# alazarteka/Self-Forcing

Measured on AMD Instinct MI355X. Metric: decoded frames/sec/node, Wan-1.3B 832x480 4-step AR rollout, higher is better.
Workload: dtype bf16

## Files before the change

self-forcing_amd/csrc/dit_forward.hip:

```cpp
#include <algorithm>
#include "sf_host.h"

int sf_internal_write_kv_indices(void* buf, int layers, int64_t global_end, int64_t local_end, void* stream);

namespace {

struct Work {
  void *x, *xn, *qkv, *q, *att, *hbuf, *cols, *headout, *sin, *etmp, *e, *e0, *ctx1, *ctx;
  void* xq;
  float* xs;
  size_t total;
};

constexpr int FP8_MAX_SEGMENTS = 8;

Work carve(const sf_model* m, void* ws, int B, int F, int lat_h, int lat_w, int groups) {
  const size_t M = (size_t)B * F * (lat_h / 2) * (lat_w / 2);
  const size_t C = m->dim, BG = (size_t)B * groups, T = (size_t)B * m->text_len;
  Carve c(ws);
  Work w;
  w.x = c.take(M * C * 2);
  w.xn = c.take(M * C * 2);
  w.qkv = c.take(M * 3 * C * 2);
  w.q = c.take(M * C * 2);
// ... 34 lines not shown
  w.t1 = c.take(R * im->clip_dim * 2);
  w.ctx = c.take(2 * R * (size_t)m->dim * 2);
  w.total = c.off;
  return w;
}

}

extern "C" size_t sf_dit_workspace_bytes(const sf_model* model, const sf_i2v_model* i2v_model, int batch, int frames, int lat_h, int lat_w,
                                         int groups) {
  if (!model || batch <= 0 || frames <= 0 || lat_h <= 0 || lat_w <= 0 || groups <= 0) return 0;
  const size_t base = carve(model, nullptr, batch, frames, lat_h, lat_w, groups).total;
  if (!i2v_model) return base;
  if (!base || i2v_model->clip_len <= 0 || i2v_model->clip_dim <= 0) return 0;
  return carve_img(model, i2v_model, nullptr, base, batch).total;
}

extern "C" int sf_dit_forward(const sf_model* m, const sf_forward_call* call, void* stream) {
  SF_CHECK(m && call, "sf_dit_forward: null argument");
  const sf_forward_args* const* ps = call->passes;
  const int np = call->n_passes;
  SF_CHECK(np == 1 || np == 2, "sf_dit_forward: one or two passes per call (n_passes=%d)", np);
  const sf_forward_args* a = ps[0];
  SF_CHECK(a && ps[np - 1], "sf_dit_forward: null argument");
  SF_CHECK(ps[np - 1]->workspace == a->workspace && ps[np - 1]->workspace_bytes == a->workspace_bytes,
           "sf_dit_forward: both passes name the same workspace (sized for 2 x batch)");
  int32_t* const cross_keys = call->cross_keys;
  float* const cross_log2w = call->cross_log2w;
  SF_CHECK((cross_keys == nullptr) == (cross_log2w == nullptr), "sf_dit_forward: cross_keys and cross_log2w come together");
  const sf_i2v_model* const im = call->i2v_model;
// ... 120 lines not shown
      void* ctx_img = (void*)bptr(iw.ctx, (size_t)R * C);
      SF_TRY(sf_layernorm_rows(ia->clip_feature, im->img_ln0_w, im->img_ln0_b, iw.t0, R, D, im->img_eps, stream));
      SF_TRY(Gemm(iw.t0, D, im->img_fc1_w, D, iw.t1, D, R, D, D).bias(im->img_fc1_b).bf16(stream));
      SF_TRY(sf_clip_gelu(iw.t1, iw.t1, (int64_t)R * D, stream));
      SF_TRY(Gemm(iw.t1, D, im->img_fc2_w, D, ctx_raw, C, R, C, D).bias(im->img_fc2_b).bf16(stream));
      SF_TRY(sf_layernorm_affine(ctx_raw, im->img_ln1_w, im->img_ln1_b, ctx_img, R, C, im->img_eps, stream));
      for (int l = 0; l < m->num_layers; ++l) {
        const sf_i2v_layer& il = im->layers_host[l];
        SF_TRY(Gemm(ctx_img, C, il.kvimg_w, C, ia->kimg_cache_host[l], C, R, C, C).bias(il.kvimg_b).bf16(stream));
        SF_TRY(sf_rmsnorm(ia->kimg_cache_host[l], C, il.norm_k_img_w, ia->kimg_cache_host[l], C, R, C, m->eps, stream));
        SF_TRY(Gemm(ctx_img, C, bptr(il.kvimg_w, (size_t)C * C), C, ia->vimg_cache_host[l], C, R, C, C).bias(bptr(il.kvimg_b, C)).bf16(stream));
      }
    }
  }

  for (int l = 0; l < m->num_layers; ++l) {
    const sf_layer_weights& lw = m->layers_host[l];
    const sf_layer_fp8& lq = f8 ? m->layers_fp8_host[l] : no_fp8;
    const void* mod = lw.modulation;
    const bool last_layer = l == m->num_layers - 1;
    SF_TRY(sf_layernorm_modulate(ws.x, ws.xn, Mt, C, m->eps, bptr(mod, 0), bptr(mod, C), bptr(ws.e0, 0), bptr(ws.e0, C), 6L * C, rpg, stream));
    SF_TRY(lin(Gemm(ws.xn, C, lw.qkv_w, C, ws.qkv, 3 * C, Mt, 3 * C, C).bias(lw.qkv_b).fp8w(lq.qkv_q, lq.qkv_s, M)));
    for (int p = 0; p < np; ++p) {
      const sf_forward_args* q = ps[p];
      const size_t roff = (size_t)p * M;
      if (q->evict > 0) {
        SF_TRY(sf_kv_evict(q->k_cache_host[l], B, q->cache_tokens, C, q->sink_tokens, q->evict, q->keep, q->evict_scratch, q->evict_scratch_bytes, stream));
        SF_TRY(sf_kv_evict(q->v_cache_host[l], B, q->cache_tokens, C, q->sink_tokens, q->evict, q->keep, q->evict_scratch, q->evict_scratch_bytes, stream));
      }
      SF_TRY(sf_qkv_norm_rope_cache(bptr(ws.qkv, roff * 3 * C), lw.norm_q_w, lw.norm_k_w, (void*)bptr(ws.q, roff * C), q->k_cache_host[l], q->v_cache_host[l],
                                    m->rope_cos, m->rope_sin, B, F, h, w, C, m->num_heads, q->cache_tokens, q->write_start, q->start_frame, m->eps, stream));
      if (q->cache_only && last_layer) continue;
      SF_TRY(Attention(bptr(ws.q, roff * C), C, (long)L * C, bptr(q->k_cache_host[l], (size_t)q->attn_start * C), bptr(q->v_cache_host[l], (size_t)q->attn_start * C),
                       C, cache_b, (void*)bptr(ws.att, roff * C), C, (long)L * C, B, m->num_heads, L, q->attn_end - q->attn_start).run(stream));
    }
    const int p0 = last_layer ? first_full : 0;
    if (p0 == np) return finish_indices();
    const size_t r0 = (size_t)p0 * M;
    const int Mr = (np - p0) * M;
    void* x = (void*)bptr(ws.x, r0 * C);
    void* xn = (void*)bptr(ws.xn, r0 * C);
    void* qb = (void*)bptr(ws.q, r0 * C);
    void* att = (void*)bptr(ws.att, r0 * C);
    void* hb = (void*)bptr(ws.hbuf, r0 * m->ffn_dim);
    const void* e0r = bptr(ws.e0, (size_t)p0 * BG * 6 * C);
    SF_TRY(lin(Gemm(att, C, lw.o_w, C, x, C, Mr, C, C).bias(lw.o_b).epi(SF_EPI_BIAS_GATE_RESID).resid(x, C)
// ... 33 lines not shown
```

self-forcing_amd/csrc/elementwise.hip:

```cpp
#include "sf_common.h"
#include "../../include/sf_hip.h"

namespace {

constexpr int ROWS_PER_BLOCK = 4;

template <int NCH>
__device__ __forceinline__ void load_row(const bf16_t* row, int lane, float (&v)[NCH][8]) {
#pragma unroll
  for (int i = 0; i < NCH; ++i) {
    const bf16x8 t = *reinterpret_cast<const bf16x8*>(row + (i * 64 + lane) * 8);
#pragma unroll
    for (int j = 0; j < 8; ++j) v[i][j] = (float)t[j];
  }
}

template <int NCH>
__device__ __forceinline__ void ln_stats(const float (&v)[NCH][8], int C, float eps, float& mean, float& rstd) {
  float s = 0.f;
#pragma unroll
  for (int i = 0; i < NCH; ++i)
#pragma unroll
    for (int j = 0; j < 8; ++j) s += v[i][j];
  mean = wave_sum(s) / (float)C;
// ... 88 lines not shown
  for (int i = 0; i < NCH; ++i)
#pragma unroll
    for (int j = 0; j < 8; ++j) q += v[i][j] * v[i][j];
  const float r = rsqrtf(wave_sum(q) / (float)C + eps);
#pragma unroll
  for (int i = 0; i < NCH; ++i) {
    const int e = (i * 64 + lane) * 8;
    const bf16x8 wt = *reinterpret_cast<const bf16x8*>(w + e);
    bf16x8 o;
#pragma unroll
    for (int j = 0; j < 8; ++j) o[j] = (bf16_t)((float)(bf16_t)(v[i][j] * r) * (float)wt[j]);
    *reinterpret_cast<bf16x8*>(out + (long)row * ldo + e) = o;
  }
}

template <int NCH>
__global__ __launch_bounds__(256) void qkv_norm_rope_cache_kernel(
    const bf16_t* __restrict__ qkv, const bf16_t* __restrict__ wq, const bf16_t* __restrict__ wk,
    bf16_t* __restrict__ q_out, bf16_t* __restrict__ k_cache, bf16_t* __restrict__ v_cache,
    const float* __restrict__ rope_cos, const float* __restrict__ rope_sin, int rows, int L, int hgt, int wid, int C,
    long cache_tokens, int write_start, int start_frame, float eps, int c0, int c1) {
  const int lane = threadIdx.x & 63;
  const int row = blockIdx.x * ROWS_PER_BLOCK + (threadIdx.x >> 6);
  if (row >= rows) return;
  const int b = row / L, t = row - b * L;
  const int fi = t / (hgt * wid), rem = t - fi * (hgt * wid);
  const int hi = rem / wid, wi = rem - hi * wid;
  const int pos_t = start_frame + fi;
  const bf16_t* src = qkv + (long)row * 3 * C;
  const long crow = ((long)b * cache_tokens + write_start + t) * C;

#pragma unroll
  for (int i = 0; i < NCH; ++i) {
    const int e = (i * 64 + lane) * 8;
    *reinterpret_cast<u32x4*>(v_cache + crow + e) = *reinterpret_cast<const u32x4*>(src + 2 * C + e);
  }

#pragma unroll
  for (int which = 0; which < 2; ++which) {
    float v[NCH][8];
    load_row<NCH>(src + which * C, lane, v);
    float q = 0.f;
#pragma unroll
    for (int i = 0; i < NCH; ++i)
#pragma unroll
      for (int j = 0; j < 8; ++j) q += v[i][j] * v[i][j];
    const float r = rsqrtf(wave_sum(q) / (float)C + eps);
    const bf16_t* wn = which ? wk : wq;
    bf16_t* dst = which ? (k_cache + crow) : (q_out + (long)row * C);
#pragma unroll
    for (int i = 0; i < NCH; ++i) {
      const int e = (i * 64 + lane) * 8;
      const bf16x8 wt = *reinterpret_cast<const bf16x8*>(wn + e);
      const int pair0 = (e & 127) >> 1;
// ... 206 lines not shown
extern "C" int sf_rmsnorm(const void* x, int ldx, const void* weight, void* out, int ldo, int M, int C, float eps,
                          void* stream) {
  SF_CHECK(x && out && weight, "sf_rmsnorm: null tensor");
  SF_CHECK(M > 0 && channels_ok(C) && ldx >= C && ldo >= C && ldx % 8 == 0 && ldo % 8 == 0, "sf_rmsnorm: unsupported shape M=%d C=%d", M, C);
  const dim3 grid((M + ROWS_PER_BLOCK - 1) / ROWS_PER_BLOCK), block(256);
  hipStream_t s = (hipStream_t)stream;
  switch (C / 512) {
#define SF_RMS_CASE(N) \
  case N: return sf_launch<&rmsnorm_kernel<N>>("sf_rmsnorm", grid, block, 0, s, (const bf16_t*)x, ldx, (const bf16_t*)weight, (bf16_t*)out, ldo, M, C, eps);
    SF_RMS_CASE(1) SF_RMS_CASE(2) SF_RMS_CASE(3) SF_RMS_CASE(4) SF_RMS_CASE(5) SF_RMS_CASE(6) SF_RMS_CASE(8) SF_RMS_CASE(10)
#undef SF_RMS_CASE
    default: SF_CHECK(false, "sf_rmsnorm: unsupported channel count %d", C);
  }
}

extern "C" int sf_qkv_norm_rope_cache(const void* qkv, const void* norm_q_w, const void* norm_k_w, void* q_out,
                                      void* k_cache, void* v_cache, const float* rope_cos, const float* rope_sin,
                                      int B, int f, int h, int w, int C, int num_heads, int64_t cache_tokens,
                                      int write_start, int start_frame, float eps, void* stream) {
  SF_CHECK(qkv && norm_q_w && norm_k_w && q_out && k_cache && v_cache && rope_cos && rope_sin, "sf_qkv_norm_rope_cache: null tensor");
  SF_CHECK(B > 0 && f > 0 && h > 0 && w > 0 && channels_ok(C), "sf_qkv_norm_rope_cache: unsupported shape");
  SF_CHECK(num_heads > 0 && C == num_heads * 128, "sf_qkv_norm_rope_cache: head_dim must be 128 (C=%d heads=%d)", C, num_heads);
  const int L = f * h * w;
  SF_CHECK(write_start >= 0 && (int64_t)write_start + L <= cache_tokens, "sf_qkv_norm_rope_cache: cache overflow: write_start=%d + L=%d > capacity=%lld",
           write_start, L, (long long)cache_tokens);
  SF_CHECK(start_frame >= 0 && start_frame + f <= 1024 && h <= 1024 && w <= 1024, "sf_qkv_norm_rope_cache: RoPE position out of the 1024-entry table");
  const int rows = B * L;
  const dim3 grid((rows + ROWS_PER_BLOCK - 1) / ROWS_PER_BLOCK), block(256);
  hipStream_t s = (hipStream_t)stream;
  const int c = 64, c1 = c / 3, c0 = c - 2 * c1;
  switch (C / 512) {
#define SF_QKV_CASE(N)                                                                                                                         \
  case N: return sf_launch<&qkv_norm_rope_cache_kernel<N>>("sf_qkv_norm_rope_cache", grid, block, 0, s, (const bf16_t*)qkv, (const bf16_t*)norm_q_w, \
                             (const bf16_t*)norm_k_w, (bf16_t*)q_out, (bf16_t*)k_cache, (bf16_t*)v_cache, rope_cos, rope_sin,                    \
                             rows, L, h, w, C, (long)cache_tokens, write_start, start_frame, eps, c0, c1);
    SF_QKV_CASE(1) SF_QKV_CASE(2) SF_QKV_CASE(3) SF_QKV_CASE(4) SF_QKV_CASE(5) SF_QKV_CASE(6) SF_QKV_CASE(8) SF_QKV_CASE(10)
#undef SF_QKV_CASE
    default: SF_CHECK(false, "sf_qkv_norm_rope_cache: unsupported channel count %d", C);
  }
}

extern "C" int sf_kv_evict(void* cache, int B, int64_t cache_tokens, int row_elems, int sink, int evict, int keep,
                           void* scratch, size_t scratch_bytes, void* stream) {
  SF_CHECK(cache && B > 0 && row_elems > 0 && (row_elems % 8) == 0, "sf_kv_evict: bad arguments");
  SF_CHECK(sink >= 0 && evict >= 0 && keep >= 0 && (int64_t)sink + evict + keep <= cache_tokens, "sf_kv_evict: window out of range");
  if (evict == 0 || keep == 0) return 0;
  const long row_b = (long)row_elems * 2;
  const long bytes = (long)keep * row_b;
  SF_CHECK(scratch && scratch_bytes >= (size_t)(bytes * B), "sf_kv_evict: scratch too small (%zu < %ld)", scratch_bytes, bytes * B);
  char* base = (char*)cache;
  const long bstride = (long)cache_tokens * row_b;
  const int gx = (int)min((long)2048, (bytes / 16 + 255) / 256);
  const dim3 grid(gx, B), block(256);
  hipStream_t s = (hipStream_t)stream;
// ... 122 lines not shown
```

self-forcing_amd/csrc/gemm_bf16.hip:

```cpp
#include <type_traits>
#include "sf_common.h"
#include "lds_dma.h"
#include "../../include/sf_hip.h"

namespace {

constexpr int BM = 128, BN = 128, BK = 64;
constexpr int GEMM_THREADS = 256;
constexpr int TILE_BYTES = BM * BK * 2;
constexpr int STAGE_BYTES = 2 * TILE_BYTES;
constexpr int GEMM_LDS = 2 * STAGE_BYTES;

struct GemmP {
  const bf16_t* a;
  const bf16_t* w;
  const bf16_t* bias;
  bf16_t* out;
  const bf16_t* resid;
  const bf16_t* gate_mod;
  const bf16_t* gate_e0;
  long gate_group_stride;
  int rows_per_group;
  int M, N, K, lda, ldw, ldo, ldr;
  int tiles_m, tiles_n;
  long a_bs, w_bs, o_bs, r_bs;
  const float* a_scale;
  const float* w_scale;
  int rows_per_seg;
};

typedef int i32x4 __attribute__((ext_vector_type(4)));
typedef int i32x8 __attribute__((ext_vector_type(8)));

__device__ __forceinline__ f32x4 mfma_f8(const bf16x8& w0, const bf16x8& w1, const bf16x8& x0, const bf16x8& x1, const f32x4& acc) {
  const i32x8 wv = __builtin_shufflevector(__builtin_bit_cast(i32x4, w0), __builtin_bit_cast(i32x4, w1), 0, 1, 2, 3, 4, 5, 6, 7);
  const i32x8 xv = __builtin_shufflevector(__builtin_bit_cast(i32x4, x0), __builtin_bit_cast(i32x4, x1), 0, 1, 2, 3, 4, 5, 6, 7);
  return __builtin_amdgcn_mfma_scale_f32_16x16x128_f8f6f4(wv, xv, acc, 0, 0, 0, 127, 0, 127);
}

template <int MT>
__device__ __forceinline__ void fp8_scale_acc(const GemmP& p, f32x4 (&acc)[MT][4], int m_base, int n_base, int lane) {
  f32x4 ws[4];
#pragma unroll
  for (int nt = 0; nt < 4; ++nt) ws[nt] = *reinterpret_cast<const f32x4*>(p.w_scale + min(n_base + nt * 16 + (lane >> 4) * 4, p.N - 4));
// ... 58 lines not shown
  __device__ __forceinline__ bf16x4 bias() const { return *reinterpret_cast<const bf16x4*>(p.bias + n); }
  __device__ __forceinline__ bf16x4 gate_mod() const { return *reinterpret_cast<const bf16x4*>(p.gate_mod + n); }
  __device__ __forceinline__ bf16x4 gate_e0() const { return *reinterpret_cast<const bf16x4*>(e0row + n); }
  __device__ __forceinline__ bf16x4 resid() const { return *reinterpret_cast<const bf16x4*>(p.resid + (long)m * p.ldr + n); }
};

struct EpiRegs {
  bf16x4 b, gm, ge, rv;
  __device__ __forceinline__ bool has_bias() const { return true; }
  __device__ __forceinline__ bf16x4 bias() const { return b; }
  __device__ __forceinline__ bf16x4 gate_mod() const { return gm; }
  __device__ __forceinline__ bf16x4 gate_e0() const { return ge; }
  __device__ __forceinline__ bf16x4 resid() const { return rv; }
};

template <int EPI, int MT>
__device__ __forceinline__ void gemm_epilogue(const GemmP& p, f32x4 (&acc)[MT][4], int mrow, int ncol) {
#pragma unroll
  for (int mt = 0; mt < MT; ++mt) {
    const int m = mrow + mt * 16;
    if (m >= p.M) continue;
    const bf16_t* e0row = nullptr;
    if (EPI == SF_EPI_BIAS_GATE_RESID) e0row = p.gate_e0 + (long)(m / p.rows_per_group) * p.gate_group_stride;
#pragma unroll
    for (int nt = 0; nt < 4; ++nt) {
      const int n = ncol + nt * 16;
      if (n >= p.N) continue;
      if (EPI == SF_EPI_F32) {
        *reinterpret_cast<f32x4*>(reinterpret_cast<float*>(p.out) + (long)m * p.ldo + n) = acc[mt][nt];
        continue;
      }
      *reinterpret_cast<bf16x4*>(p.out + (long)m * p.ldo + n) = epi_math<EPI>(acc[mt][nt], EpiLoads{p, m, n, e0row});
    }
  }
}

template <int EPI, int MT>
__device__ __forceinline__ void gemm_epilogue_lds(const GemmP& p, f32x4 (&acc)[MT][4], int m_base, int n_base, char* wbuf, int lane) {
  const int r16 = lane & 15, cg = lane >> 4;
  constexpr bool GATE = EPI == SF_EPI_BIAS_GATE_RESID;
  constexpr bool RESID = EPI == SF_EPI_BIAS_RESID || EPI == SF_EPI_BIAS_GATE_RESID;
  const bf16x4 zero4 = {(bf16_t)0.f, (bf16_t)0.f, (bf16_t)0.f, (bf16_t)0.f};
  int ncol[4];
  bf16x4 bias_v[4], gm_v[4];
#pragma unroll
  for (int nt = 0; nt < 4; ++nt) {
    ncol[nt] = min(n_base + nt * 16 + cg * 4, p.N - 4);
    bias_v[nt] = zero4;
    gm_v[nt] = zero4;
  }
  if (p.bias) {
#pragma unroll
// ... 21 lines not shown
#pragma unroll
    for (int i = 0; i < MB; ++i) {
      if (m0 + i >= MT) break;
      const int row = (m0 + i) * 16 + r16;
#pragma unroll
      for (int nt = 0; nt < 4; ++nt) {
        const int col = nt * 16 + cg * 4;
        const bf16x4 o = epi_math<EPI>(acc[m0 + i][nt], EpiRegs{bias_v[nt], gm_v[nt], ge[i][nt], rv[i][nt]});
        const int chunk = (col >> 3) ^ (row & 7);
        *reinterpret_cast<bf16x4*>(wbuf + row * 128 + (chunk << 4) + (col & 4) * 2) = o;
      }
    }
  }
  __builtin_amdgcn_s_waitcnt(0xc07f);
  const int rr = lane >> 3, ch = lane & 7;
#pragma unroll
  for (int i = 0; i < 2 * MT; ++i) {
    const int row = i * 8 + rr;
    const int m = m_base + row, n = n_base + ch * 8;
    const bf16x8 v = *reinterpret_cast<const bf16x8*>(wbuf + row * 128 + ((ch ^ (row & 7)) << 4));
    if (m < p.M && n < p.N) *reinterpret_cast<bf16x8*>(p.out + (long)m * p.ldo + n) = v;
  }
}

template <int EPI, bool F8>
__global__ __launch_bounds__(GEMM_THREADS, 2) void gemm_bf16_kernel(GemmP p) {
  extern __shared__ __attribute__((aligned(16))) char smem[];
  const int tid = threadIdx.x;
  const int lane = tid & 63;
  const int wave = __builtin_amdgcn_readfirstlane(tid >> 6);

  if (blockIdx.y) {
    const long bz = blockIdx.y;
    p.a += bz * p.a_bs; p.w += bz * p.w_bs;
    if (EPI == SF_EPI_F32) p.out = reinterpret_cast<bf16_t*>(reinterpret_cast<float*>(p.out) + bz * p.o_bs); else p.out += bz * p.o_bs;
    if (p.resid) p.resid += bz * p.r_bs;
  }
  int tm, tn;
  gemm_tile_of<8>(p, tm, tn);
  const int m0 = tm * BM, n0 = tn * BN;

  const bf16_t* a_src[4];
  const bf16_t* w_src[4];
#pragma unroll
  for (int i = 0; i < 4; ++i) {
    const int r = (wave * 4 + i) * 8 + (lane >> 3);
    const int c = (lane & 7) ^ ((r >> 1) & 7);
// ... 78 lines not shown
      __builtin_amdgcn_sched_barrier(0);
    }
#pragma unroll
    for (int mt = 0; mt < 4; ++mt)
#pragma unroll
      for (int nt = 0; nt < 4; ++nt)
        acc[mt][nt] = __builtin_amdgcn_mfma_f32_16x16x32_bf16(wf1[nt], xf1[mt], acc[mt][nt], 0, 0, 0);
    __builtin_amdgcn_sched_barrier(0);
    __syncthreads();
  }

  if constexpr (F8) fp8_scale_acc<4>(p, acc, m0 + wr * 64, n0 + wc * 64, lane);
  const int mrow = m0 + wr * 64 + (lane & 15);
  const int ncol = n0 + wc * 64 + (lane >> 4) * 4;
  if (EPI != SF_EPI_F32 && (p.N & 7) == 0 && (p.ldo & 7) == 0)
    gemm_epilogue_lds<EPI, 4>(p, acc, m0 + wr * 64, n0 + wc * 64, smem + wave * 8192, lane);
  else
    gemm_epilogue<EPI, 4>(p, acc, mrow, ncol);
}


constexpr int PP_THREADS = 512;

__device__ __forceinline__ void pp_end_load_segment() {
  __builtin_amdgcn_s_waitcnt(0xc07f);
  __builtin_amdgcn_sched_barrier(0);
  __builtin_amdgcn_s_barrier();
  __builtin_amdgcn_sched_barrier(0);
}

template <bool F8, int R0, int NQ, int MT, int NA>
__device__ __forceinline__ void pp_cluster(f32x4 (&acc)[MT][4], const bf16x8 (&af)[NA][2], const bf16x8 (&bfr)[4][2], int c0) {
  __builtin_amdgcn_s_setprio(1);
// ... 16 lines not shown
  __builtin_amdgcn_sched_barrier(0);
  __builtin_amdgcn_s_barrier();
  __builtin_amdgcn_sched_barrier(0);
}

template <int MT>
struct PPCfg {
  static constexpr int BM = 32 * MT;
  static constexpr int A_BYTES = BM * 128;
  static constexpr int B_BYTES = 256 * 128;
  static constexpr int STAGE = A_BYTES + B_BYTES;
  static constexpr int LDS = 2 * STAGE;
  static constexpr int PA = (2 * MT + 7) / 8;
};

template <int EPI, int MT, bool F8>
__global__ __launch_bounds__(PP_THREADS) void gemm_pp_kernel(GemmP p) {
  using Cfg = PPCfg<MT>;
  constexpr int BMp = Cfg::BM, PA = Cfg::PA;
  constexpr int HQA = (MT + 1) / 2, HQB = MT / 2;
  extern __shared__ __attribute__((aligned(16))) char smem[];
  const int tid = threadIdx.x;
  const int lane = tid & 63;
  const int wave = __builtin_amdgcn_readfirstlane(tid >> 6);
  const int grp = wave >> 2, wc = wave & 3;

  int tm, tn;
  gemm_tile_of<(MT >= 6 ? 4 : 8)>(p, tm, tn);
  const int m0 = tm * BMp, n0 = tn * 256;

  const bf16_t* a_src[2][PA];
// ... 95 lines not shown
      asm volatile("s_waitcnt vmcnt(4)" ::: "memory");
    } else {
      asm volatile("s_waitcnt vmcnt(0)" ::: "memory");
    }
    pp_end_load_segment();
    cluster(Q1, 0);
  }
  if (grp == 0) __builtin_amdgcn_s_barrier();
#ifdef SF_STAMP
  if (stamp && (tid & 255) == 0) stamp[2] = __builtin_amdgcn_s_memtime();
#endif

  const int m_base = m0 + grp * (BMp / 2), n_base = n0 + wc * 64;
  if constexpr (F8) fp8_scale_acc<MT>(p, acc, m_base, n_base, lane);
  if ((p.N & 7) == 0 && (p.ldo & 7) == 0)
    gemm_epilogue_lds<EPI, MT>(p, acc, m_base, n_base, smem + wave * (MT * 2048), lane);
  else
    gemm_epilogue<EPI, MT>(p, acc, m_base + (lane & 15), n_base + (lane >> 4) * 4);
#ifdef SF_STAMP
  asm volatile("s_waitcnt vmcnt(0)" ::: "memory");
  if (stamp && (tid & 255) == 0) { stamp[3] = __builtin_amdgcn_s_memtime(); stamp[5] = __builtin_amdgcn_s_memrealtime(); }
#endif
}

constexpr int PP2_A = 128 * 128, PP2_B = 256 * 128;
constexpr int PP2_LDS = 3 * (PP2_A + PP2_B);

template <int EPI, bool F8>
__global__ __launch_bounds__(PP_THREADS) void gemm_pp2_kernel(GemmP p) {
  extern __shared__ __attribute__((aligned(16))) char smem[];
  const int tid = threadIdx.x;
  const int lane = tid & 63;
  const int wave = __builtin_amdgcn_readfirstlane(tid >> 6);
  const int grp = wave >> 2, wc = wave & 3;

  int tm, tn;
  gemm_tile_of<8>(p, tm, tn);
  const int m0 = tm * 128, n0 = tn * 256;

  const bf16_t* a_src[2];
  const bf16_t* w_src[4];
#pragma unroll
  for (int i = 0; i < 2; ++i) {
// ... 62 lines not shown
    if (more2) {
      dma_b(nslot, kt + 2);
      asm volatile("s_waitcnt vmcnt(6)" ::: "memory");
    } else {
      asm volatile("s_waitcnt vmcnt(0)" ::: "memory");
    }
    pp_end_load_segment();
    cluster(2);
    slot = slot == 2 ? 0 : slot + 1;
  }
  if (grp == 0) __builtin_amdgcn_s_barrier();

  const int m_base = m0 + grp * 64, n_base = n0 + wc * 64;
  if constexpr (F8) fp8_scale_acc<4>(p, acc, m_base, n_base, lane);
  if ((p.N & 7) == 0 && (p.ldo & 7) == 0)
    gemm_epilogue_lds<EPI, 4>(p, acc, m_base, n_base, smem + wave * 8192, lane);
  else
    gemm_epilogue<EPI, 4>(p, acc, m_base + (lane & 15), n_base + (lane >> 4) * 4);
}

template <class F>
int with_epilogue(int epilogue, const char* name, F&& f) {
  switch (epilogue) {
    case SF_EPI_BIAS: return f(std::integral_constant<int, SF_EPI_BIAS>{});
    case SF_EPI_BIAS_GELU: return f(std::integral_constant<int, SF_EPI_BIAS_GELU>{});
    case SF_EPI_BIAS_RESID: return f(std::integral_constant<int, SF_EPI_BIAS_RESID>{});
    case SF_EPI_BIAS_GATE_RESID: return f(std::integral_constant<int, SF_EPI_BIAS_GATE_RESID>{});
    default: SF_CHECK(false, "%s: unknown epilogue %d", name, epilogue);
  }
}

template <int MT, bool F8>
int launch_pp(GemmP& p, int epilogue, const char* name, hipStream_t s) {
  using Cfg = PPCfg<MT>;
  p.tiles_m = (p.M + Cfg::BM - 1) / Cfg::BM;
  p.tiles_n = (p.N + 255) / 256;
  return with_epilogue(epilogue, name, [&](auto epi) {
    return sf_launch<&gemm_pp_kernel<decltype(epi)::value, MT, F8>, Cfg::LDS>(name, dim3(p.tiles_m * p.tiles_n), dim3(PP_THREADS), Cfg::LDS, s, p);
  });
}

template <bool F8>
int launch_pp2(GemmP& p, int epilogue, const char* name, hipStream_t s) {
  p.tiles_m = (p.M + 127) / 128;
  p.tiles_n = (p.N + 255) / 256;
  return with_epilogue(epilogue, name, [&](auto epi) {
    return sf_launch<&gemm_pp2_kernel<decltype(epi)::value, F8>, PP2_LDS>(name, dim3(p.tiles_m * p.tiles_n), dim3(PP_THREADS), PP2_LDS, s, p);
  });
}

struct PPStructure {
  int st, rows;
  double rel;
  int (*launch)(GemmP&, int, const char*, hipStream_t);
};
template <bool F8>
constexpr PPStructure PP_STRUCTURES[] = {{SF_GEMM_PP256, 256, 1.00, launch_pp<8, F8>},
                                         {SF_GEMM_PP224, 224, 1.02, launch_pp<7, F8>},
                                         {SF_GEMM_PP192, 192, 1.05, launch_pp<6, F8>},
                                         {SF_GEMM_PP128, 128, 1.14, launch_pp2<F8>}};

int check_args(const sf_gemm_args* a, const char* name, int bk) {
// ... 30 lines not shown
        const double cost = (double)((tiles + 255) / 256) * (c.rows / 256.0 * c.rel + 0.04);
        if (cost < best - 1e-9) { best = cost; st = c.st; }
      }
    }
  }
  if (pp_ok)
    for (const auto& c : PP_STRUCTURES<F8>)
      if (c.st == st) return c.launch(p, a->epilogue, name, s);
  const int batch = a->batch > 1 ? a->batch : 1;
  p.a_bs = a->a_bstride; p.w_bs = a->w_bstride; p.o_bs = a->o_bstride; p.r_bs = a->r_bstride;
  SF_CHECK(batch == 1 || (a->a_bstride % 8 == 0 && a->w_bstride % 8 == 0 && a->o_bstride % 4 == 0 && a->r_bstride % 4 == 0),
           "%s: batch strides must keep 16-byte (operands) / 8-byte (output) alignment", name);
  const dim3 grid(p.tiles_m * p.tiles_n, batch), block(GEMM_THREADS);
  if (a->epilogue != SF_EPI_F32)
    return with_epilogue(a->epilogue, name, [&](auto epi) {
      return sf_launch<&gemm_bf16_kernel<decltype(epi)::value, F8>>(name, grid, block, GEMM_LDS, s, p);
    });
  if constexpr (F8) {
    SF_CHECK(false, "%s: the raw fp32 epilogue is bf16-only", name);
  } else {
    SF_CHECK((uintptr_t)a->out % 16 == 0, "%s: fp32 output must be 16-byte aligned", name);
    return sf_launch<&gemm_bf16_kernel<SF_EPI_F32, false>>(name, grid, block, GEMM_LDS, s, p);
  }
}

void fill_params(const sf_gemm_args* a, GemmP& p, int unit) {
  p.a = (const bf16_t*)a->a; p.w = (const bf16_t*)a->w; p.bias = (const bf16_t*)a->bias;
  p.out = (bf16_t*)a->out; p.resid = (const bf16_t*)a->resid;
  p.gate_mod = (const bf16_t*)a->gate_mod; p.gate_e0 = (const bf16_t*)a->gate_e0;
  p.gate_group_stride = a->gate_group_stride; p.rows_per_group = a->rows_per_group;
  p.M = a->M; p.N = a->N; p.K = a->K / unit; p.lda = a->lda / unit; p.ldw = a->ldw / unit; p.ldo = a->ldo; p.ldr = a->ldr;
  p.tiles_n = (a->N + BN - 1) / BN;
  p.tiles_m = (a->M + BM - 1) / BM;
  p.a_scale = nullptr; p.w_scale = nullptr; p.rows_per_seg = 1;
}

}

extern "C" int sf_gemm_bf16(const sf_gemm_args* a, void* stream) {
  if (const int rc = check_args(a, "sf_gemm_bf16", BK)) return rc;
  GemmP p;
  fill_params(a, p, 1);
  return run_gemm<false>(a, p, "sf_gemm_bf16", (hipStream_t)stream);
}

extern "C" int sf_gemm_fp8(const sf_gemm_args* a, const float* a_scale, int rows_per_segment, const float* w_scale, void* stream) {
  if (const int rc = check_args(a, "sf_gemm_fp8", 2 * BK)) return rc;
  SF_CHECK(a->batch <= 1, "sf_gemm_fp8: batched products are bf16-only");
  SF_CHECK(a_scale && w_scale && rows_per_segment > 0, "sf_gemm_fp8: needs a_scale, w_scale and rows_per_segment > 0");
  SF_CHECK((uintptr_t)w_scale % 16 == 0, "sf_gemm_fp8: w_scale must be 16-byte aligned");
  GemmP p;
  fill_params(a, p, 2);
  p.a_scale = a_scale; p.w_scale = w_scale; p.rows_per_seg = rows_per_segment;
  return run_gemm<true>(a, p, "sf_gemm_fp8", (hipStream_t)stream);
}
```

self-forcing_amd/csrc/sf_host.h:

```cpp
#pragma once
#include <cstring>
#include "sf_common.h"
#include "../../include/sf_hip.h"

inline int sf_hip_ok(hipError_t e, const char* who, const char* what) {
  SF_CHECK(e == hipSuccess, "%s: %s failed: %s", who, what, hipGetErrorString(e));
  return 0;
}

struct Carve {
  char* base;
  size_t off;
  explicit Carve(void* p) : base((char*)p), off(0) {}
  char* take(size_t bytes) {
    char* r = base ? base + off : nullptr;
    off += (bytes + 255) & ~(size_t)255;
    return r;
  }
};

struct Gemm {
  sf_gemm_args g;
  const void* wq = nullptr;
  const float* w_scale = nullptr;
  int rows_per_segment = 0;
  Gemm(const void* a, int lda, const void* w, int ldw, void* out, int ldo, int M, int N, int K) {
    memset(&g, 0, sizeof(g));
    g.a = a; g.lda = lda; g.w = w; g.ldw = ldw; g.out = out; g.ldo = ldo; g.M = M; g.N = N; g.K = K;
    g.epilogue = SF_EPI_BIAS;
    g.rows_per_group = 1;
  }
  Gemm& bias(const void* b) { g.bias = b; return *this; }
  Gemm& epi(int e) { g.epilogue = e; return *this; }
  Gemm& resid(const void* r, int ldr) { g.resid = r; g.ldr = ldr; return *this; }
  Gemm& gate(const void* gate_mod, const void* gate_e0, long group_stride, int rows_per_group) {
    g.gate_mod = gate_mod; g.gate_e0 = gate_e0; g.gate_group_stride = group_stride; g.rows_per_group = rows_per_group;
    return *this;
  }
  Gemm& batch(int n, long a_bstride, long w_bstride, long o_bstride) {
    g.batch = n; g.a_bstride = a_bstride; g.w_bstride = w_bstride; g.o_bstride = o_bstride;
    return *this;
  }
  Gemm& fp8w(const void* w_e4m3, const float* scale, int rows_per_seg) {
    wq = w_e4m3; w_scale = scale; rows_per_segment = rows_per_seg;
    return *this;
  }
  int bf16(void* stream) const { return sf_gemm_bf16(&g, stream); }
  int fp8(const void* aq, const float* a_scale, void* stream) const {
    sf_gemm_args q = g;
    q.a = aq; q.lda = g.K; q.w = wq;
    return sf_gemm_fp8(&q, a_scale, rows_per_segment, w_scale, stream);
  }
};

struct Attention {
  sf_attention_args a;
  Attention(const void* q, long q_stride, long q_bstride, const void* k, const void* v, long kv_stride, long kv_bstride, void* out,
            long o_stride, long o_bstride, int B, int H, int Lq, int Lk) {
    memset(&a, 0, sizeof(a));
    a.q = q; a.q_stride = q_stride; a.q_bstride = q_bstride;
    a.k = k; a.v = v; a.kv_stride = kv_stride; a.kv_bstride = kv_bstride;
    a.out = out; a.o_stride = o_stride; a.o_bstride = o_bstride;
    a.B = B; a.H = H; a.Lq = Lq; a.Lk = Lk;
// ... 8 lines not shown
```

Measured before the change: 95.83.

## Write V directly into KV cache from QKV GEMM epilogue

```diff
diff --git a/self-forcing_amd/csrc/dit_forward.hip b/self-forcing_amd/csrc/dit_forward.hip
--- a/self-forcing_amd/csrc/dit_forward.hip
+++ b/self-forcing_amd/csrc/dit_forward.hip
@@ -1,9 +1,16 @@
 #include <algorithm>
+#include <atomic>
 #include "sf_host.h"
 
 int sf_internal_write_kv_indices(void* buf, int layers, int64_t global_end, int64_t local_end, void* stream);
+int sf_internal_qk_norm_rope_cache(const void* qkv, const void* norm_q_w, const void* norm_k_w, void* q_out, void* k_cache, const float* rope_cos,
+                                   const float* rope_sin, int B, int f, int h, int w, int C, int num_heads, int64_t cache_tokens, int write_start,
+                                   int start_frame, float eps, int skip_q, void* stream);
 
 namespace {
+
+std::atomic<int> v_direct_on{1};
+std::atomic<long long> v_direct_calls{0};
 
 struct Work {
   void *x, *xn, *qkv, *q, *att, *hbuf, *cols, *headout, *sin, *etmp, *e, *e0, *ctx1, *ctx;
@@ -72,6 +79,11 @@
   if (!i2v_model) return base;
   if (!base || i2v_model->clip_len <= 0 || i2v_model->clip_dim <= 0) return 0;
   return carve_img(model, i2v_model, nullptr, base, batch).total;
+}
+
+extern "C" long long sf_internal_set_v_direct(int mode) {
+  if (mode == 0 || mode == 1) v_direct_on.store(mode);
+  return v_direct_calls.load();
 }
 
 extern "C" int sf_dit_forward(const sf_model* m, const sf_forward_call* call, void* stream) {
@@ -222,13 +234,40 @@
     }
   }
 
+  bool v_direct = v_direct_on.load() != 0 && !f8 && !im && np * B <= SF_GEMM_SPLIT_MAX_SEGS;
+  for (int p = 0; p < np && v_direct; ++p) {
+    if (ps[p]->evict > 0) v_direct = false;
+    for (int p2 = p + 1; p2 < np; ++p2)
+      if ((int64_t)ps[p2]->write_start + L > ps[p]->attn_start && ps[p2]->write_start < ps[p]->attn_end) v_direct = false;
+  }
+  for (int l = 0; l < m->num_layers && v_direct; ++l)
+    if ((uintptr_t)a->v_cache_host[l] % 16 != 0) v_direct = false;
+  sf_gemm_split v_split = {};
+  if (v_direct) {
+    v_split.ldo2 = C; v_split.n_split = 2 * C; v_split.seg_rows = L; v_split.n_segs = np * B;
+    for (int p = 0; p < np; ++p)
+      for (int b = 0; b < B; ++b) v_split.seg_row0[p * B + b] = (int64_t)b * a->cache_tokens + ps[p]->write_start;
+    v_direct_calls.fetch_add(1);
+  }
+  const bool kv_only_last = v_direct && first_full == np && C % 256 == 0;
+
   for (int l = 0; l < m->num_layers; ++l) {
     const sf_layer_weights& lw = m->layers_host[l];
     const sf_layer_fp8& lq = f8 ? m->layers_fp8_host[l] : no_fp8;
     const void* mod = lw.modulation;
     const bool last_layer = l == m->num_layers - 1;
+    const bool kv_only = kv_only_last && last_layer;
     SF_TRY(sf_layernorm_modulate(ws.x, ws.xn, Mt, C, m->eps, bptr(mod, 0), bptr(mod, C), bptr(ws.e0, 0), bptr(ws.e0, C), 6L * C, rpg, stream));
-    SF_TRY(lin(Gemm(ws.xn, C, lw.qkv_w, C, ws.qkv, 3 * C, Mt, 3 * C, C).bias(lw.qkv_b).fp8w(lq.qkv_q, lq.qkv_s, M)));
+    if (v_direct) {
+      v_split.out2 = a->v_cache_host[l];
+      v_split.n_split = kv_only ? C : 2 * C;
+      if (kv_only)
+        SF_TRY(Gemm(ws.xn, C, bptr(lw.qkv_w, (size_t)C * C), C, (void*)bptr(ws.qkv, C), 3 * C, Mt, 2 * C, C).bias(bptr(lw.qkv_b, C)).split(v_split).bf16(stream));
+      else
+        SF_TRY(Gemm(ws.xn, C, lw.qkv_w, C, ws.qkv, 3 * C, Mt, 3 * C, C).bias(lw.qkv_b).split(v_split).bf16(stream));
+    } else {
+      SF_TRY(lin(Gemm(ws.xn, C, lw.qkv_w, C, ws.qkv, 3 * C, Mt, 3 * C, C).bias(lw.qkv_b).fp8w(lq.qkv_q, lq.qkv_s, M)));
+    }
     for (int p = 0; p < np; ++p) {
       const sf_forward_args* q = ps[p];
       const size_t roff = (size_t)p * M;
@@ -236,8 +275,12 @@
         SF_TRY(sf_kv_evict(q->k_cache_host[l], B, q->cache_tokens, C, q->sink_tokens, q->evict, q->keep, q->evict_scratch, q->evict_scratch_bytes, stream));
         SF_TRY(sf_kv_evict(q->v_cache_host[l], B, q->cache_tokens, C, q->sink_tokens, q->evict, q->keep, q->evict_scratch, q->evict_scratch_bytes, stream));
       }
-      SF_TRY(sf_qkv_norm_rope_cache(bptr(ws.qkv, roff * 3 * C), lw.norm_q_w, lw.norm_k_w, (void*)bptr(ws.q, roff * C), q->k_cache_host[l], q->v_cache_host[l],
-                                    m->rope_cos, m->rope_sin, B, F, h, w, C, m->num_heads, q->cache_tokens, q->write_start, q->start_frame, m->eps, stream));
+      if (v_direct)
+        SF_TRY(sf_internal_qk_norm_rope_cache(bptr(ws.qkv, roff * 3 * C), lw.norm_q_w, lw.norm_k_w, (void*)bptr(ws.q, roff * C), q->k_cache_host[l], m->rope_cos,
+                                              m->rope_sin, B, F, h, w, C, m->num_heads, q->cache_tokens, q->write_start, q->start_frame, m->eps, kv_only, stream));
+      else
+        SF_TRY(sf_qkv_norm_rope_cache(bptr(ws.qkv, roff * 3 * C), lw.norm_q_w, lw.norm_k_w, (void*)bptr(ws.q, roff * C), q->k_cache_host[l], q->v_cache_host[l],
+                                      m->rope_cos, m->rope_sin, B, F, h, w, C, m->num_heads, q->cache_tokens, q->write_start, q->start_frame, m->eps, stream));
       if (q->cache_only && last_layer) continue;
       SF_TRY(Attention(bptr(ws.q, roff * C), C, (long)L * C, bptr(q->k_cache_host[l], (size_t)q->attn_start * C), bptr(q->v_cache_host[l], (size_t)q->attn_start * C),
                        C, cache_b, (void*)bptr(ws.att, roff * C), C, (long)L * C, B, m->num_heads, L, q->attn_end - q->attn_start).run(stream));
diff --git a/self-forcing_amd/csrc/elementwise.hip b/self-forcing_amd/csrc/elementwise.hip
--- a/self-forcing_amd/csrc/elementwise.hip
+++ b/self-forcing_amd/csrc/elementwise.hip
@@ -126,7 +126,7 @@
   }
 }
 
-template <int NCH>
+template <int NCH, bool COPY_V = true, bool WRITE_Q = true>
 __global__ __launch_bounds__(256) void qkv_norm_rope_cache_kernel(
     const bf16_t* __restrict__ qkv, const bf16_t* __restrict__ wq, const bf16_t* __restrict__ wk,
     bf16_t* __restrict__ q_out, bf16_t* __restrict__ k_cache, bf16_t* __restrict__ v_cache,
@@ -142,14 +142,16 @@
   const bf16_t* src = qkv + (long)row * 3 * C;
   const long crow = ((long)b * cache_tokens + write_start + t) * C;
 
-#pragma unroll
-  for (int i = 0; i < NCH; ++i) {
-    const int e = (i * 64 + lane) * 8;
-    *reinterpret_cast<u32x4*>(v_cache + crow + e) = *reinterpret_cast<const u32x4*>(src + 2 * C + e);
-  }
-
-#pragma unroll
-  for (int which = 0; which < 2; ++which) {
+  if constexpr (COPY_V) {
+#pragma unroll
+    for (int i = 0; i < NCH; ++i) {
+      const int e = (i * 64 + lane) * 8;
+      *reinterpret_cast<u32x4*>(v_cache + crow + e) = *reinterpret_cast<const u32x4*>(src + 2 * C + e);
+    }
+  }
+
+#pragma unroll
+  for (int which = WRITE_Q ? 0 : 1; which < 2; ++which) {
     float v[NCH][8];
     load_row<NCH>(src + which * C, lane, v);
     float q = 0.f;
@@ -386,30 +388,53 @@
   }
 }
 
+namespace {
+int qkv_norm_rope_cache_launch(int mode, const char* name, const void* qkv, const void* norm_q_w, const void* norm_k_w, void* q_out, void* k_cache,
+                               void* v_cache, const float* rope_cos, const float* rope_sin, int B, int f, int h, int w, int C, int num_heads,
+                               int64_t cache_tokens, int write_start, int start_frame, float eps, void* stream) {
+  SF_CHECK(qkv && norm_q_w && norm_k_w && (q_out || mode == 2) && k_cache && (v_cache || mode != 0) && rope_cos && rope_sin, "%s: null tensor", name);
+  SF_CHECK(B > 0 && f > 0 && h > 0 && w > 0 && channels_ok(C), "%s: unsupported shape", name);
+  SF_CHECK(num_heads > 0 && C == num_heads * 128, "%s: head_dim must be 128 (C=%d heads=%d)", name, C, num_heads);
+  const int L = f * h * w;
+  SF_CHECK(write_start >= 0 && (int64_t)write_start + L <= cache_tokens, "%s: cache overflow: write_start=%d + L=%d > capacity=%lld", name,
+           write_start, L, (long long)cache_tokens);
+  SF_CHECK(start_frame >= 0 && start_frame + f <= 1024 && h <= 1024 && w <= 1024, "%s: RoPE position out of the 1024-entry table", name);
+  const int rows = B * L;
+  const dim3 grid((rows + ROWS_PER_BLOCK - 1) / ROWS_PER_BLOCK), block(256);
+  hipStream_t s = (hipStream_t)stream;
+  const int c = 64, c1 = c / 3, c0 = c - 2 * c1;
+#define SF_QKV_LAUNCH(...)                                                                                                                  \
+  sf_launch<&qkv_norm_rope_cache_kernel<__VA_ARGS__>>(name, grid, block, 0, s, (const bf16_t*)qkv, (const bf16_t*)norm_q_w, (const bf16_t*)norm_k_w, \
+                                                      (bf16_t*)q_out, (bf16_t*)k_cache, (bf16_t*)v_cache, rope_cos, rope_sin, rows, L, h, w, C,      \
+                                                      (long)cache_tokens, write_start, start_frame, eps, c0, c1)
+#define SF_QKV_CASE(N)                                \
+  case N:                                             \
+    if (mode == 0) return SF_QKV_LAUNCH(N);           \
+    if (mode == 1) return SF_QKV_LAUNCH(N, false);    \
+    return SF_QKV_LAUNCH(N, false, false);
+  switch (C / 512) {
+    SF_QKV_CASE(1) SF_QKV_CASE(2) SF_QKV_CASE(3) SF_QKV_CASE(4) SF_QKV_CASE(5) SF_QKV_CASE(6) SF_QKV_CASE(8) SF_QKV_CASE(10)
+#undef SF_QKV_CASE
+#undef SF_QKV_LAUNCH
+    default: SF_CHECK(false, "%s: unsupported channel count %d", name, C);
+  }
+}
+}
+
 extern "C" int sf_qkv_norm_rope_cache(const void* qkv, const void* norm_q_w, const void* norm_k_w, void* q_out,
                                       void* k_cache, void* v_cache, const float* rope_cos, const float* rope_sin,
                                       int B, int f, int h, int w, int C, int num_heads, int64_t cache_tokens,
                                       int write_start, int start_frame, float eps, void* stream) {
-  SF_CHECK(qkv && norm_q_w && norm_k_w && q_out && k_cache && v_cache && rope_cos && rope_sin, "sf_qkv_norm_rope_cache: null tensor");
-  SF_CHECK(B > 0 && f > 0 && h > 0 && w > 0 && channels_ok(C), "sf_qkv_norm_rope_cache: unsupported shape");
-  SF_CHECK(num_heads > 0 && C == num_heads * 128, "sf_qkv_norm_rope_cache: head_dim must be 128 (C=%d heads=%d)", C, num_heads);
-  const int L = f * h * w;
-  SF_CHECK(write_start >= 0 && (int64_t)write_start + L <= cache_tokens, "sf_qkv_norm_rope_cache: cache overflow: write_start=%d + L=%d > capacity=%lld",
-           write_start, L, (long long)cache_tokens);
-  SF_CHECK(start_frame >= 0 && start_frame + f <= 1024 && h <= 1024 && w <= 1024, "sf_qkv_norm_rope_cache: RoPE position out of the 1024-entry table");
-  const int rows = B * L;
-  const dim3 grid((rows + ROWS_PER_BLOCK - 1) / ROWS_PER_BLOCK), block(256);
-  hipStream_t s = (hipStream_t)stream;
-  const int c = 64, c1 = c / 3, c0 = c - 2 * c1;
-  switch (C / 512) {
-#define SF_QKV_CASE(N)                                                                                                                         \
-  case N: return sf_launch<&qkv_norm_rope_cache_kernel<N>>("sf_qkv_norm_rope_cache", grid, block, 0, s, (const bf16_t*)qkv, (const bf16_t*)norm_q_w, \
-                             (const bf16_t*)norm_k_w, (bf16_t*)q_out, (bf16_t*)k_cache, (bf16_t*)v_cache, rope_cos, rope_sin,                    \
-                             rows, L, h, w, C, (long)cache_tokens, write_start, start_frame, eps, c0, c1);
-    SF_QKV_CASE(1) SF_QKV_CASE(2) SF_QKV_CASE(3) SF_QKV_CASE(4) SF_QKV_CASE(5) SF_QKV_CASE(6) SF_QKV_CASE(8) SF_QKV_CASE(10)
-#undef SF_QKV_CASE
-    default: SF_CHECK(false, "sf_qkv_norm_rope_cache: unsupported channel count %d", C);
-  }
+  return qkv_norm_rope_cache_launch(0, "sf_qkv_norm_rope_cache", qkv, norm_q_w, norm_k_w, q_out, k_cache, v_cache, rope_cos, rope_sin, B, f, h, w, C, num_heads,
+                                    cache_tokens, write_start, start_frame, eps, stream);
+}
+
+__attribute__((visibility("hidden"))) int sf_internal_qk_norm_rope_cache(const void* qkv, const void* norm_q_w, const void* norm_k_w, void* q_out, void* k_cache,
+                                                                         const float* rope_cos, const float* rope_sin, int B, int f, int h, int w, int C,
+                                                                         int num_heads, int64_t cache_tokens, int write_start, int start_frame, float eps,
+                                                                         int skip_q, void* stream) {
+  return qkv_norm_rope_cache_launch(skip_q ? 2 : 1, "sf_internal_qk_norm_rope_cache", qkv, norm_q_w, norm_k_w, q_out, k_cache, nullptr, rope_cos, rope_sin, B, f,
+                                    h, w, C, num_heads, cache_tokens, write_start, start_frame, eps, stream);
 }
 
 extern "C" int sf_kv_evict(void* cache, int B, int64_t cache_tokens, int row_elems, int sink, int evict, int keep,
diff --git a/self-forcing_amd/csrc/gemm_bf16.hip b/self-forcing_amd/csrc/gemm_bf16.hip
--- a/self-forcing_amd/csrc/gemm_bf16.hip
+++ b/self-forcing_amd/csrc/gemm_bf16.hip
@@ -1,6 +1,7 @@
 #include <type_traits>
 #include "sf_common.h"
 #include "lds_dma.h"
+#include "sf_host.h"
 #include "../../include/sf_hip.h"
 
 namespace {
@@ -27,7 +28,19 @@
   const float* a_scale;
   const float* w_scale;
   int rows_per_seg;
+  bf16_t* out2;
+  int ldo2, n_split, seg_rows;
+  long seg_delta[SF_GEMM_SPLIT_MAX_SEGS];
 };
+
+__device__ __forceinline__ long split_delta(const GemmP& p, int m) {
+  long d = p.seg_delta[0];
+#pragma unroll
+  for (int s = 1; s < SF_GEMM_SPLIT_MAX_SEGS; ++s)
+    if (m >= s * p.seg_rows) d = p.seg_delta[s];
+  return d;
+}
+__device__ __forceinline__ long split_row(const GemmP& p, int m) { return m + split_delta(p, m); }
 
 typedef int i32x4 __attribute__((ext_vector_type(4)));
 typedef int i32x8 __attribute__((ext_vector_type(8)));
@@ -116,8 +129,10 @@
   __device__ __forceinline__ bf16x4 resid() const { return rv; }
 };
 
-template <int EPI, int MT>
+template <int EPI, int MT, bool SPLIT>
 __device__ __forceinline__ void gemm_epilogue(const GemmP& p, f32x4 (&acc)[MT][4], int mrow, int ncol) {
+  static_assert(!SPLIT || EPI != SF_EPI_F32, "the split is built for the bf16 epilogues");
+  const bool to2 = SPLIT && ncol >= p.n_split;
 #pragma unroll
   for (int mt = 0; mt < MT; ++mt) {
     const int m = mrow + mt * 16;
@@ -132,12 +147,19 @@
         *reinterpret_cast<f32x4*>(reinterpret_cast<float*>(p.out) + (long)m * p.ldo + n) = acc[mt][nt];
         continue;
       }
-      *reinterpret_cast<bf16x4*>(p.out + (long)m * p.ldo + n) = epi_math<EPI>(acc[mt][nt], EpiLoads{p, m, n, e0row});
-    }
-  }
-}
-
-template <int EPI, int MT>
+      const bf16x4 o = epi_math<EPI>(acc[mt][nt], EpiLoads{p, m, n, e0row});
+      if constexpr (SPLIT) {
+        if (to2) {
+          *reinterpret_cast<bf16x4*>(p.out2 + split_row(p, m) * p.ldo2 + (n - p.n_split)) = o;
+          continue;
+        }
+      }
+      *reinterpret_cast<bf16x4*>(p.out + (long)m * p.ldo + n) = o;
+    }
+  }
+}
+
+template <int EPI, int MT, bool SPLIT>
 __device__ __forceinline__ void gemm_epilogue_lds(const GemmP& p, f32x4 (&acc)[MT][4], int m_base, int n_base, char* wbuf, int lane) {
   const int r16 = lane & 15, cg = lane >> 4;
   constexpr bool GATE = EPI == SF_EPI_BIAS_GATE_RESID;
@@ -189,23 +211,34 @@
   }
   __builtin_amdgcn_s_waitcnt(0xc07f);
   const int rr = lane >> 3, ch = lane & 7;
+  const bool to2 = SPLIT && n_base >= p.n_split;
 #pragma unroll
   for (int i = 0; i < 2 * MT; ++i) {
     const int row = i * 8 + rr;
     const int m = m_base + row, n = n_base + ch * 8;
     const bf16x8 v = *reinterpret_cast<const bf16x8*>(wbuf + row * 128 + ((ch ^ (row & 7)) << 4));
+    if constexpr (SPLIT) {
+      if (to2) {
+        const int g0 = m_base + i * 8;
+        const long d0 = split_delta(p, g0), d1 = split_delta(p, g0 + 7);
+        long d = d0;
+        if (d0 != d1 || p.seg_rows < 8) d = split_delta(p, m);
+        if (m < p.M && n < p.N) *reinterpret_cast<bf16x8*>(p.out2 + (d * p.ldo2 - p.n_split) + ((long)m * p.ldo2 + n)) = v;
+        continue;
+      }
+    }
     if (m < p.M && n < p.N) *reinterpret_cast<bf16x8*>(p.out + (long)m * p.ldo + n) = v;
   }
 }
 
-template <int EPI, bool F8>
+template <int EPI, bool F8, bool SPLIT>
 __global__ __launch_bounds__(GEMM_THREADS, 2) void gemm_bf16_kernel(GemmP p) {
   extern __shared__ __attribute__((aligned(16))) char smem[];
   const int tid = threadIdx.x;
   const int lane = tid & 63;
   const int wave = __builtin_amdgcn_readfirstlane(tid >> 6);
 
-  if (blockIdx.y) {
+  if (!SPLIT && blockIdx.y) {
     const long bz = blockIdx.y;
     p.a += bz * p.a_bs; p.w += bz * p.w_bs;
     if (EPI == SF_EPI_F32) p.out = reinterpret_cast<bf16_t*>(reinterpret_cast<float*>(p.out) + bz * p.o_bs); else p.out += bz * p.o_bs;
@@ -314,9 +347,9 @@
   const int mrow = m0 + wr * 64 + (lane & 15);
   const int ncol = n0 + wc * 64 + (lane >> 4) * 4;
   if (EPI != SF_EPI_F32 && (p.N & 7) == 0 && (p.ldo & 7) == 0)
-    gemm_epilogue_lds<EPI, 4>(p, acc, m0 + wr * 64, n0 + wc * 64, smem + wave * 8192, lane);
+    gemm_epilogue_lds<EPI, 4, SPLIT>(p, acc, m0 + wr * 64, n0 + wc * 64, smem + wave * 8192, lane);
   else
-    gemm_epilogue<EPI, 4>(p, acc, mrow, ncol);
+    gemm_epilogue<EPI, 4, SPLIT>(p, acc, mrow, ncol);
 }
 
 
@@ -363,7 +396,7 @@
   static constexpr int PA = (2 * MT + 7) / 8;
 };
 
-template <int EPI, int MT, bool F8>
+template <int EPI, int MT, bool F8, bool SPLIT>
 __global__ __launch_bounds__(PP_THREADS) void gemm_pp_kernel(GemmP p) {
   using Cfg = PPCfg<MT>;
   constexpr int BMp = Cfg::BM, PA = Cfg::PA;
@@ -489,9 +522,9 @@
   const int m_base = m0 + grp * (BMp / 2), n_base = n0 + wc * 64;
   if constexpr (F8) fp8_scale_acc<MT>(p, acc, m_base, n_base, lane);
   if ((p.N & 7) == 0 && (p.ldo & 7) == 0)
-    gemm_epilogue_lds<EPI, MT>(p, acc, m_base, n_base, smem + wave * (MT * 2048), lane);
+    gemm_epilogue_lds<EPI, MT, SPLIT>(p, acc, m_base, n_base, smem + wave * (MT * 2048), lane);
   else
-    gemm_epilogue<EPI, MT>(p, acc, m_base + (lane & 15), n_base + (lane >> 4) * 4);
+    gemm_epilogue<EPI, MT, SPLIT>(p, acc, m_base + (lane & 15), n_base + (lane >> 4) * 4);
 #ifdef SF_STAMP
   asm volatile("s_waitcnt vmcnt(0)" ::: "memory");
   if (stamp && (tid & 255) == 0) { stamp[3] = __builtin_amdgcn_s_memtime(); stamp[5] = __builtin_amdgcn_s_memrealtime(); }
@@ -501,7 +534,7 @@
 constexpr int PP2_A = 128 * 128, PP2_B = 256 * 128;
 constexpr int PP2_LDS = 3 * (PP2_A + PP2_B);
 
-template <int EPI, bool F8>
+template <int EPI, bool F8, bool SPLIT>
 __global__ __launch_bounds__(PP_THREADS) void gemm_pp2_kernel(GemmP p) {
   extern __shared__ __attribute__((aligned(16))) char smem[];
   const int tid = threadIdx.x;
@@ -594,9 +627,9 @@
   const int m_base = m0 + grp * 64, n_base = n0 + wc * 64;
   if constexpr (F8) fp8_scale_acc<4>(p, acc, m_base, n_base, lane);
   if ((p.N & 7) == 0 && (p.ldo & 7) == 0)
-    gemm_epilogue_lds<EPI, 4>(p, acc, m_base, n_base, smem + wave * 8192, lane);
+    gemm_epilogue_lds<EPI, 4, SPLIT>(p, acc, m_base, n_base, smem + wave * 8192, lane);
   else
-    gemm_epilogue<EPI, 4>(p, acc, m_base + (lane & 15), n_base + (lane >> 4) * 4);
+    gemm_epilogue<EPI, 4, SPLIT>(p, acc, m_base + (lane & 15), n_base + (lane >> 4) * 4);
 }
 
 template <class F>
@@ -616,7 +649,10 @@
   p.tiles_m = (p.M + Cfg::BM - 1) / Cfg::BM;
   p.tiles_n = (p.N + 255) / 256;
   return with_epilogue(epilogue, name, [&](auto epi) {
-    return sf_launch<&gemm_pp_kernel<decltype(epi)::value, MT, F8>, Cfg::LDS>(name, dim3(p.tiles_m * p.tiles_n), dim3(PP_THREADS), Cfg::LDS, s, p);
+    if constexpr (!F8)
+      if (p.out2)
+        return sf_launch<&gemm_pp_kernel<decltype(epi)::value, MT, false, true>, Cfg::LDS>(name, dim3(p.tiles_m * p.tiles_n), dim3(PP_THREADS), Cfg::LDS, s, p);
+    return sf_launch<&gemm_pp_kernel<decltype(epi)::value, MT, F8, false>, Cfg::LDS>(name, dim3(p.tiles_m * p.tiles_n), dim3(PP_THREADS), Cfg::LDS, s, p);
   });
 }
 
@@ -625,7 +661,10 @@
   p.tiles_m = (p.M + 127) / 128;
   p.tiles_n = (p.N + 255) / 256;
   return with_epilogue(epilogue, name, [&](auto epi) {
-    return sf_launch<&gemm_pp2_kernel<decltype(epi)::value, F8>, PP2_LDS>(name, dim3(p.tiles_m * p.tiles_n), dim3(PP_THREADS), PP2_LDS, s, p);
+    if constexpr (!F8)
+      if (p.out2)
+        return sf_launch<&gemm_pp2_kernel<decltype(epi)::value, false, true>, PP2_LDS>(name, dim3(p.tiles_m * p.tiles_n), dim3(PP_THREADS), PP2_LDS, s, p);
+    return sf_launch<&gemm_pp2_kernel<decltype(epi)::value, F8, false>, PP2_LDS>(name, dim3(p.tiles_m * p.tiles_n), dim3(PP_THREADS), PP2_LDS, s, p);
   });
 }
 
@@ -686,13 +725,15 @@
   const dim3 grid(p.tiles_m * p.tiles_n, batch), block(GEMM_THREADS);
   if (a->epilogue != SF_EPI_F32)
     return with_epilogue(a->epilogue, name, [&](auto epi) {
-      return sf_launch<&gemm_bf16_kernel<decltype(epi)::value, F8>>(name, grid, block, GEMM_LDS, s, p);
+      if constexpr (!F8)
+        if (p.out2) return sf_launch<&gemm_bf16_kernel<decltype(epi)::value, false, true>>(name, grid, block, GEMM_LDS, s, p);
+      return sf_launch<&gemm_bf16_kernel<decltype(epi)::value, F8, false>>(name, grid, block, GEMM_LDS, s, p);
     });
   if constexpr (F8) {
     SF_CHECK(false, "%s: the raw fp32 epilogue is bf16-only", name);
   } else {
     SF_CHECK((uintptr_t)a->out % 16 == 0, "%s: fp32 output must be 16-byte aligned", name);
-    return sf_launch<&gemm_bf16_kernel<SF_EPI_F32, false>>(name, grid, block, GEMM_LDS, s, p);
+    return sf_launch<&gemm_bf16_kernel<SF_EPI_F32, false, false>>(name, grid, block, GEMM_LDS, s, p);
   }
 }
 
@@ -705,6 +746,8 @@
   p.tiles_n = (a->N + BN - 1) / BN;
   p.tiles_m = (a->M + BM - 1) / BM;
   p.a_scale = nullptr; p.w_scale = nullptr; p.rows_per_seg = 1;
+  p.out2 = nullptr; p.ldo2 = 0; p.n_split = 0; p.seg_rows = 1;
+  for (long& d : p.seg_delta) d = 0;
 }
 
 }
@@ -714,6 +757,39 @@
   GemmP p;
   fill_params(a, p, 1);
   return run_gemm<false>(a, p, "sf_gemm_bf16", (hipStream_t)stream);
+}
+
+extern "C" __attribute__((visibility("hidden"))) int sf_internal_gemm_split(const sf_gemm_args* a, const sf_gemm_split* sp, void* stream) {
+  const char* name = "sf_internal_gemm_split";
+  if (const int rc = check_args(a, name, BK)) return rc;
+  SF_CHECK(sp && sp->out2, "%s: null second destination", name);
+  SF_CHECK(a->batch <= 1 && a->epilogue != SF_EPI_F32, "%s: unbatched products with a bf16 epilogue only", name);
+  SF_CHECK(sp->n_split > 0 && sp->n_split % 256 == 0 && sp->n_split < a->N, "%s: n_split=%d must be a multiple of 256 inside N=%d", name, sp->n_split, a->N);
+  SF_CHECK((a->N - sp->n_split) % 8 == 0, "%s: N - n_split = %d must be a multiple of 8", name, a->N - sp->n_split);
+  SF_CHECK(sp->ldo2 >= a->N - sp->n_split && sp->ldo2 % 8 == 0, "%s: ldo2=%d must be a multiple of 8, at least N - n_split", name, sp->ldo2);
+  SF_CHECK((uintptr_t)sp->out2 % 16 == 0, "%s: out2 must be 16-byte aligned", name);
+  SF_CHECK(sp->n_segs >= 1 && sp->n_segs <= SF_GEMM_SPLIT_MAX_SEGS && sp->seg_rows > 0, "%s: 1..%d segments of at least one row (n_segs=%d seg_rows=%d)", name,
+           SF_GEMM_SPLIT_MAX_SEGS, sp->n_segs, sp->seg_rows);
+  SF_CHECK((int64_t)sp->n_segs * sp->seg_rows >= a->M, "%s: %d segments of %d rows do not cover M=%d", name, sp->n_segs, sp->seg_rows, a->M);
+  SF_CHECK((int64_t)sp->seg_rows * SF_GEMM_SPLIT_MAX_SEGS <= INT32_MAX, "%s: seg_rows=%d too large", name, sp->seg_rows);
+  GemmP p;
+  fill_params(a, p, 1);
+  p.out2 = (bf16_t*)sp->out2; p.ldo2 = sp->ldo2; p.n_split = sp->n_split; p.seg_rows = sp->seg_rows;
+  for (int s = 0; s < SF_GEMM_SPLIT_MAX_SEGS; ++s) {
+    const int t = s < sp->n_segs ? s : sp->n_segs - 1;
+    SF_CHECK(sp->seg_row0[t] >= 0, "%s: negative destination row", name);
+    p.seg_delta[s] = (long)sp->seg_row0[t] - (long)t * sp->seg_rows;
+  }
+  return run_gemm<false>(a, p, name, (hipStream_t)stream);
+}
+
+extern "C" int sf_internal_gemm_split_flat(const sf_gemm_args* a, void* out2, int ldo2, int n_split, int seg_rows, int n_segs, const int64_t* seg_row0,
+                                           void* stream) {
+  SF_CHECK(seg_row0 && n_segs >= 1 && n_segs <= SF_GEMM_SPLIT_MAX_SEGS, "sf_internal_gemm_split_flat: 1..%d segments", SF_GEMM_SPLIT_MAX_SEGS);
+  sf_gemm_split sp = {};
+  sp.out2 = out2; sp.ldo2 = ldo2; sp.n_split = n_split; sp.seg_rows = seg_rows; sp.n_segs = n_segs;
+  for (int s = 0; s < n_segs; ++s) sp.seg_row0[s] = seg_row0[s];
+  return sf_internal_gemm_split(a, &sp, stream);
 }
 
 extern "C" int sf_gemm_fp8(const sf_gemm_args* a, const float* a_scale, int rows_per_segment, const float* w_scale, void* stream) {
diff --git a/self-forcing_amd/csrc/sf_host.h b/self-forcing_amd/csrc/sf_host.h
--- a/self-forcing_amd/csrc/sf_host.h
+++ b/self-forcing_amd/csrc/sf_host.h
@@ -19,11 +19,20 @@
   }
 };
 
+constexpr int SF_GEMM_SPLIT_MAX_SEGS = 8;
+struct sf_gemm_split {
+  void* out2;
+  int ldo2, n_split, seg_rows, n_segs;
+  int64_t seg_row0[SF_GEMM_SPLIT_MAX_SEGS];
+};
+extern "C" __attribute__((visibility("hidden"))) int sf_internal_gemm_split(const sf_gemm_args* a, const sf_gemm_split* sp, void* stream);
+
 struct Gemm {
   sf_gemm_args g;
   const void* wq = nullptr;
   const float* w_scale = nullptr;
   int rows_per_segment = 0;
+  sf_gemm_split sp = {};
   Gemm(const void* a, int lda, const void* w, int ldw, void* out, int ldo, int M, int N, int K) {
     memset(&g, 0, sizeof(g));
     g.a = a; g.lda = lda; g.w = w; g.ldw = ldw; g.out = out; g.ldo = ldo; g.M = M; g.N = N; g.K = K;
@@ -45,8 +54,10 @@
     wq = w_e4m3; w_scale = scale; rows_per_segment = rows_per_seg;
     return *this;
   }
-  int bf16(void* stream) const { return sf_gemm_bf16(&g, stream); }
+  Gemm& split(const sf_gemm_split& s) { sp = s; return *this; }
+  int bf16(void* stream) const { return sp.out2 ? sf_internal_gemm_split(&g, &sp, stream) : sf_gemm_bf16(&g, stream); }
   int fp8(const void* aq, const float* a_scale, void* stream) const {
+    SF_CHECK(!sp.out2, "Gemm: the split is bf16-only");
     sf_gemm_args q = g;
     q.a = aq; q.lda = g.K; q.w = wq;
     return sf_gemm_fp8(&q, a_scale, rows_per_segment, w_scale, stream);
```

Result: no change. 96.09, median of 6 (+0.3%).
